# Sunscreen-tech/spf

Measured on NVIDIA B200. Metric: circuit_bootstraps_per_sec, higher is better.
Workload: dtype f64

## Files before the change

### spf_b200/csrc/kernels.cuh

```cuda
#pragma once
#include <cuda_runtime.h>

#include "team_ops.cuh"

namespace spf {

__device__ __forceinline__ void tmem_ld16(uint32_t (&r)[16], uint32_t taddr);
__device__ __forceinline__ void tmem_st16(uint32_t taddr, const uint32_t (&r)[16]);
__device__ __forceinline__ void tmem_wait_ld();
__device__ __forceinline__ void tmem_wait_st();

struct DevCx {
  static constexpr bool kTmemTwiddles = false;
  int u;
  int bar;
  uint32_t rp_taddr;
  __device__ __forceinline__ void sync() const {
    asm volatile("bar.sync %0, 64;" ::"r"(bar) : "memory");
  }
  __device__ __forceinline__ void rp_store(const uint64_t (&rp)[32]) const {
#pragma unroll
    for (int c = 0; c < 4; c++) {
      uint32_t r[16];
#pragma unroll
      for (int i = 0; i < 8; i++) { r[2 * i] = (uint32_t)rp[8 * c + i]; r[2 * i + 1] = (uint32_t)(rp[8 * c + i] >> 32); }
      tmem_st16(rp_taddr + 16 * c, r);
    }
    tmem_wait_st();
  }
  __device__ __forceinline__ void rp_load(uint64_t (&rp)[32]) const {
    uint32_t r[4][16];
#pragma unroll
    for (int c = 0; c < 4; c++) tmem_ld16(r[c], rp_taddr + 16 * c);
    tmem_wait_ld();
#pragma unroll
    for (int c = 0; c < 4; c++)
#pragma unroll
      for (int i = 0; i < 8; i++) rp[8 * c + i] = ((uint64_t)r[c][2 * i + 1] << 32) | r[c][2 * i];
  }
};

struct DevTables {
  const C2* T1;
  const C2* T2;
};

__device__ __forceinline__ void load_tables(C2* sT1, C2* sT2, const DevTables& t) {
  for (int i = threadIdx.x; i < kT1Elems; i += blockDim.x) sT1[i] = t.T1[i];
  for (int i = threadIdx.x; i < kT2Elems; i += blockDim.x) sT2[i] = t.T2[i];
  __syncthreads();
}

constexpr int kTableBytes = (kT1Elems + kT2Elems) * 16;

__device__ __forceinline__ void pdl_launch_dependents() { asm volatile("griddepcontrol.launch_dependents;" ::: "memory"); }
__device__ __forceinline__ void pdl_wait() { asm volatile("griddepcontrol.wait;" ::: "memory"); }
__device__ __forceinline__ void prefetch_l2(const void* p) { asm volatile("prefetch.global.L2 [%0];" ::"l"(p)); }

#ifndef SPF_PBS_PAIRS
#define SPF_PBS_PAIRS 3
#endif
#ifndef SPF_PBS_TRANSIENT
#define SPF_PBS_TRANSIENT 1
#endif
#ifndef SPF_PBS_TWOBUF
#define SPF_PBS_TWOBUF 0
#endif
constexpr int kPbsPairs = SPF_PBS_PAIRS;
constexpr int kPbsPairBytes = (SPF_PBS_TRANSIENT ? 0 : 2 * kN * 8) + (SPF_PBS_TWOBUF ? 4 : 2) * kXBuf * 16;
constexpr int kPbsTmemOwn0 = 64;
constexpr int kPbsTmemF0 = kPbsTmemOwn0 + 64 * kPbsPairs;
constexpr int kPbsTmemFPairs = (512 - kPbsTmemF0) / 64 < kPbsPairs ? (512 - kPbsTmemF0) / 64 : kPbsPairs;
constexpr int kPbsFParkBytes = (kPbsPairs - kPbsTmemFPairs) * 2 * kTeam * 16 * 16;
#ifndef SPF_PBS_RING
#define SPF_PBS_RING (!SPF_PBS_TWOBUF)
#endif
static_assert(!SPF_PBS_RING || SPF_PBS_TRANSIENT, "the BSK ring lives in the shared memory the transient accumulator frees");
#ifndef SPF_PBS_RING_STAGES
#define SPF_PBS_RING_STAGES 3
#endif
constexpr int kRingStages = SPF_PBS_RING_STAGES;
constexpr int kRingChunkElems = 2 * kM;
constexpr int kRingChunkBytes = kRingChunkElems * 16;
constexpr bool kPbsTablesInRing = SPF_PBS_RING && kRingStages == 4;
#ifndef SPF_PBS_PAIR_SHIFT
#define SPF_PBS_PAIR_SHIFT 0
#endif
constexpr int kPbsPairOff = (kPbsTablesInRing ? 0 : kTableBytes) + SPF_PBS_PAIR_SHIFT;
constexpr int kPbsRingOff = kPbsPairOff + kPbsPairs * kPbsPairBytes + kPbsFParkBytes;
constexpr int kPbsTablesOff = kPbsTablesInRing ? kPbsRingOff + 3 * kRingChunkBytes : 0;
constexpr int kPbsRingBytes = SPF_PBS_RING ? kRingStages * kRingChunkBytes + 64 : 0;
constexpr int kPbsSmem = kPbsRingOff + kPbsRingBytes;
static_assert(kPbsSmem <= 232448, "pbs_kernel shared memory");

#ifndef SPF_PBS_TMEM_T1
#define SPF_PBS_TMEM_T1 1
#endif
#ifndef SPF_PBS_TMEM_T2
#define SPF_PBS_TMEM_T2 1
#endif
#ifndef SPF_PBS_TMEM_F
#define SPF_PBS_TMEM_F 1
#endif
#ifndef SPF_PBS_TMEM_OWN
#define SPF_PBS_TMEM_OWN 1
#endif

__device__ __forceinline__ void tmem_ld16(uint32_t (&r)[16], uint32_t taddr) {
  asm volatile(
      "tcgen05.ld.sync.aligned.32x32b.x16.b32 {%0, %1, %2, %3, %4, %5, %6, %7, %8, %9, %10, %11, %12, %13, %14, %15}, [%16];"
      : "=r"(r[0]), "=r"(r[1]), "=r"(r[2]), "=r"(r[3]), "=r"(r[4]), "=r"(r[5]), "=r"(r[6]), "=r"(r[7]), "=r"(r[8]),
        "=r"(r[9]), "=r"(r[10]), "=r"(r[11]), "=r"(r[12]), "=r"(r[13]), "=r"(r[14]), "=r"(r[15])
      : "r"(taddr));
}
__device__ __forceinline__ void tmem_st4(uint32_t taddr, uint32_t a, uint32_t b, uint32_t c, uint32_t d) {
  asm volatile("tcgen05.st.sync.aligned.32x32b.x4.b32 [%0], {%1, %2, %3, %4};" ::"r"(taddr), "r"(a), "r"(b), "r"(c), "r"(d)
               : "memory");
}
__device__ __forceinline__ void tmem_st2(uint32_t taddr, uint32_t a, uint32_t b) {
  asm volatile("tcgen05.st.sync.aligned.32x32b.x2.b32 [%0], {%1, %2};" ::"r"(taddr), "r"(a), "r"(b) : "memory");
}
__device__ __forceinline__ void tmem_wait_ld() { asm volatile("tcgen05.wait::ld.sync.aligned;" ::: "memory"); }
__device__ __forceinline__ void tmem_wait_st() { asm volatile("tcgen05.wait::st.sync.aligned;" ::: "memory"); }

constexpr int kPbsTmemCols = 512;
__device__ __forceinline__ void tmem_ld8(uint32_t (&r)[8], uint32_t taddr) {
  asm volatile("tcgen05.ld.sync.aligned.32x32b.x8.b32 {%0, %1, %2, %3, %4, %5, %6, %7}, [%8];"
               : "=r"(r[0]), "=r"(r[1]), "=r"(r[2]), "=r"(r[3]), "=r"(r[4]), "=r"(r[5]), "=r"(r[6]), "=r"(r[7])
               : "r"(taddr));
}
__device__ __forceinline__ void tmem_st8(uint32_t taddr, const uint32_t (&r)[8]) {
  asm volatile("tcgen05.st.sync.aligned.32x32b.x8.b32 [%0], {%1, %2, %3, %4, %5, %6, %7, %8};" ::"r"(taddr), "r"(r[0]), "r"(r[1]),
               "r"(r[2]), "r"(r[3]), "r"(r[4]), "r"(r[5]), "r"(r[6]), "r"(r[7])
               : "memory");
}
__device__ __forceinline__ void tmem_st16(uint32_t taddr, const uint32_t (&r)[16]) {
  asm volatile(
      "tcgen05.st.sync.aligned.32x32b.x16.b32 [%0], {%1, %2, %3, %4, %5, %6, %7, %8, %9, %10, %11, %12, %13, %14, %15, %16};"
      ::"r"(taddr), "r"(r[0]), "r"(r[1]), "r"(r[2]), "r"(r[3]), "r"(r[4]), "r"(r[5]), "r"(r[6]), "r"(r[7]), "r"(r[8]),
        "r"(r[9]), "r"(r[10]), "r"(r[11]), "r"(r[12]), "r"(r[13]), "r"(r[14]), "r"(r[15])
      : "memory");
}

__device__ __forceinline__ uint32_t smem_u32(const void* p) { return (uint32_t)__cvta_generic_to_shared(p); }
__device__ __forceinline__ void mbar_wait_trap(uint32_t bar, uint32_t parity) {
  unsigned long long t_start = 0;
  for (int spin = 0;; spin++) {
    uint32_t ok;
#if SPF_MBAR_HINT
    asm volatile("{\n\t.reg .pred p;\n\tmbarrier.try_wait.parity.shared::cta.b64 p, [%1], %2, %3;\n\tselp.u32 %0, 1, 0, p;\n\t}"
                 : "=r"(ok) : "r"(bar), "r"(parity), "r"((uint32_t)SPF_MBAR_HINT) : "memory");
#else
    asm volatile("{\n\t.reg .pred p;\n\tmbarrier.try_wait.parity.shared::cta.b64 p, [%1], %2;\n\tselp.u32 %0, 1, 0, p;\n\t}"
                 : "=r"(ok) : "r"(bar), "r"(parity) : "memory");
#endif
    if (ok) return;
    if ((spin & 1023) == 1023) {
      unsigned long long now;
      asm volatile("mov.u64 %0, %%globaltimer;" : "=l"(now));
      if (t_start == 0) t_start = now;
      else if (now - t_start > 2000000000ull) __trap();
    }
  }
}
static_assert(!SPF_PBS_TRANSIENT || SPF_PBS_TMEM_OWN, "the transient accumulator image needs the tensor-memory own copy");
static_assert(!kPbsTablesInRing || SPF_PBS_TMEM_T1, "four ring stages overlay the twiddle tables: the twiddles must live in tensor memory");

#ifndef SPF_PBS_CHUNKED
#define SPF_PBS_CHUNKED 1
#endif
#ifndef SPF_PBS_READER_T2
#define SPF_PBS_READER_T2 1
#endif
#ifndef SPF_PBS_INT_CONV
#define SPF_PBS_INT_CONV 0
#endif
#ifndef SPF_PBS_FST2
#define SPF_PBS_FST2 1
#endif
#ifndef SPF_PBS_EARLY_REL
#define SPF_PBS_EARLY_REL 0
#endif
#ifndef SPF_PBS_RING_FENCE
#define SPF_PBS_RING_FENCE 1
#endif
#ifndef SPF_MBAR_HINT
#define SPF_MBAR_HINT 0
#endif
#ifndef SPF_PBS_FRND_CONV
#define SPF_PBS_FRND_CONV 0
#endif
#ifndef SPF_PBS_TW_PIPE
#define SPF_PBS_TW_PIPE 0
#endif
#ifndef SPF_PBS_FUSED_ST
#define SPF_PBS_FUSED_ST 0
#endif
#ifndef SPF_PBS_TMEM_X1
#define SPF_PBS_TMEM_X1 0
#endif
__device__ __forceinline__ void tmem_ld256x4(uint32_t* r, uint32_t taddr) {
  asm volatile(
      "tcgen05.ld.sync.aligned.16x256b.x4.b32 {%0, %1, %2, %3, %4, %5, %6, %7, %8, %9, %10, %11, %12, %13, %14, %15}, [%16];"
      : "=r"(r[0]), "=r"(r[1]), "=r"(r[2]), "=r"(r[3]), "=r"(r[4]), "=r"(r[5]), "=r"(r[6]), "=r"(r[7]), "=r"(r[8]),
        "=r"(r[9]), "=r"(r[10]), "=r"(r[11]), "=r"(r[12]), "=r"(r[13]), "=r"(r[14]), "=r"(r[15])
      : "r"(taddr));
}
__device__ __forceinline__ void tmem_st256x4(uint32_t taddr, const uint32_t* r) {
  asm volatile(
      "tcgen05.st.sync.aligned.16x256b.x4.b32 [%0], {%1, %2, %3, %4, %5, %6, %7, %8, %9, %10, %11, %12, %13, %14, %15, %16};"
      ::"r"(taddr), "r"(r[0]), "r"(r[1]), "r"(r[2]), "r"(r[3]), "r"(r[4]), "r"(r[5]), "r"(r[6]), "r"(r[7]), "r"(r[8]),
        "r"(r[9]), "r"(r[10]), "r"(r[11]), "r"(r[12]), "r"(r[13]), "r"(r[14]), "r"(r[15])
      : "memory");
}
__device__ __forceinline__ void tmem_ld16p(uint32_t* r, uint32_t taddr) {
  asm volatile(
      "tcgen05.ld.sync.aligned.32x32b.x16.b32 {%0, %1, %2, %3, %4, %5, %6, %7, %8, %9, %10, %11, %12, %13, %14, %15}, [%16];"
      : "=r"(r[0]), "=r"(r[1]), "=r"(r[2]), "=r"(r[3]), "=r"(r[4]), "=r"(r[5]), "=r"(r[6]), "=r"(r[7]), "=r"(r[8]),
        "=r"(r[9]), "=r"(r[10]), "=r"(r[11]), "=r"(r[12]), "=r"(r[13]), "=r"(r[14]), "=r"(r[15])
      : "r"(taddr));
}
__device__ __forceinline__ void tmem_st16p(uint32_t taddr, const uint32_t* r) {
  asm volatile(
      "tcgen05.st.sync.aligned.32x32b.x16.b32 [%0], {%1, %2, %3, %4, %5, %6, %7, %8, %9, %10, %11, %12, %13, %14, %15, %16};"
      ::"r"(taddr), "r"(r[0]), "r"(r[1]), "r"(r[2]), "r"(r[3]), "r"(r[4]), "r"(r[5]), "r"(r[6]), "r"(r[7]), "r"(r[8]),
        "r"(r[9]), "r"(r[10]), "r"(r[11]), "r"(r[12]), "r"(r[13]), "r"(r[14]), "r"(r[15])
      : "memory");
}
__device__ __forceinline__ constexpr int x1_unit1(int k, int c) { return (k >> 2) + 4 * (c + 2 * (k & 3)); }
__device__ __forceinline__ constexpr int x1_unit2(int e, int klo, int c) { return klo + 4 * (c + 2 * e); }
__device__ __forceinline__ constexpr int x1_reg256(int b, int eh, int ch, int cg, int w) { return 16 * (2 * b + ch) + w + 2 * eh + 4 * cg; }
__device__ __forceinline__ constexpr int x1_reg_r1(int e, int klo, int c, int w) {
  return x1_reg256(e >> 1, e & 1, klo >> 1, c + 2 * (klo & 1), w);
}
__device__ __forceinline__ constexpr int x1_reg_r2(int e, int ep, int c, int w) {
  return x1_reg256(ep >> 1, ep & 1, e >> 1, c + 2 * (e & 1), w);
}
__device__ __forceinline__ void x1_ld256(uint32_t (&r)[64], uint32_t ta) {
  tmem_ld256x4(r, ta); tmem_ld256x4(r + 16, ta + 32); tmem_ld256x4(r + 32, ta + (16u << 16)); tmem_ld256x4(r + 48, ta + 32 + (16u << 16));
}
__device__ __forceinline__ void x1_st256(uint32_t ta, const uint32_t (&r)[64]) {
  tmem_st256x4(ta, r); tmem_st256x4(ta + 32, r + 16); tmem_st256x4(ta + (16u << 16), r + 32); tmem_st256x4(ta + 32 + (16u << 16), r + 48);
}
__device__ __forceinline__ void x1_ld32(uint32_t (&r)[64], uint32_t ta) {
  tmem_ld16p(r, ta); tmem_ld16p(r + 16, ta + 16); tmem_ld16p(r + 32, ta + 32); tmem_ld16p(r + 48, ta + 48);
}
__device__ __forceinline__ void x1_st32(uint32_t ta, const uint32_t (&r)[64]) {
  tmem_st16p(ta, r); tmem_st16p(ta + 16, r + 16); tmem_st16p(ta + 32, r + 32); tmem_st16p(ta + 48, r + 48);
}
struct DevPairCx {
  static constexpr bool kTransient = SPF_PBS_TRANSIENT != 0;
  static constexpr bool kChunked = SPF_PBS_CHUNKED != 0;
  static constexpr bool kFusedStores = SPF_PBS_FUSED_ST != 0;
  static __device__ __forceinline__ void sts_c2(C2* p, C2 v) {
    asm volatile("st.shared.v2.f64 [%0], {%1, %2};" ::"r"((uint32_t)__cvta_generic_to_shared(p)), "d"(v.x), "d"(v.y) : "memory");
  }
  __device__ __forceinline__ void sts(C2* p, C2 v) const { sts_c2(p, v); }
  template <bool CONJ>
  __device__ __forceinline__ void t1_mul_store(C2 (&v)[16], const C2* T1, C2* buf) const {
#pragma unroll
    for (int g = 0; g < 4; g++) {
      uint32_t r[16];
      tmem_ld16(r, t1_taddr + 16 * g);
      tmem_wait_ld();
#pragma unroll
      for (int i = 0; i < 4; i++) {
        const C2 w{__hiloint2double((int)r[4 * i + 1], (int)r[4 * i]), __hiloint2double((int)r[4 * i + 3], (int)r[4 * i + 2])};
        const int k = 4 * g + i;
        v[k] = CONJ ? cmul_conj(v[k], w) : cmul(v[k], w);
        sts_c2(buf + k * kXPad + u, v[k]);
      }
    }
  }
  template <bool CONJ>
  __device__ __forceinline__ void t2_mul_store(C2 (&v)[16], const C2* T2, C2* buf) const {
    const int k1 = u & 15, q = u >> 4;
#pragma unroll
    for (int k2 = 0; k2 < 16; k2++) {
      if (k2) v[k2] = CONJ ? cmul_conj(v[k2], T2[q * kT2Pad + k2]) : cmul(v[k2], T2[q * kT2Pad + k2]);
      sts_c2(buf + k1 * kXPad + q + 4 * k2, v[k2]);
    }
  }
  static constexpr bool kTmemX1 = SPF_PBS_TMEM_X1 != 0;
  __device__ __forceinline__ int time_index() const { return kTmemX1 ? x1_time_index(u) : u; }
  __device__ __forceinline__ void x1_fwd(C2 (&v)[16]) const {
    uint32_t r[64], s[64];
#pragma unroll
    for (int k = 0; k < 16; k++) {
      r[2 * x1_unit1(k, 0)] = (uint32_t)__double2loint(v[k].x); r[2 * x1_unit1(k, 0) + 1] = (uint32_t)__double2hiint(v[k].x);
      r[2 * x1_unit1(k, 1)] = (uint32_t)__double2loint(v[k].y); r[2 * x1_unit1(k, 1) + 1] = (uint32_t)__double2hiint(v[k].y);
    }
    x1_st32(f_taddr, r);
    tmem_wait_st();
    x1_ld256(s, f_taddr);
    tmem_wait_ld();
#pragma unroll
    for (int e = 0; e < 4; e++)
#pragma unroll
      for (int klo = 0; klo < 4; klo++)
#pragma unroll
        for (int c = 0; c < 2; c++)
#pragma unroll
          for (int w = 0; w < 2; w++) r[2 * x1_unit2(e, klo, c) + w] = s[x1_reg_r1(e, klo, c, w)];
    x1_st32(f_taddr, r);
    tmem_wait_st();
    x1_ld256(s, f_taddr);
    tmem_wait_ld();
#pragma unroll
    for (int e = 0; e < 4; e++)
#pragma unroll
      for (int ep = 0; ep < 4; ep++) {
        v[4 * e + ep].x = __hiloint2double((int)s[x1_reg_r2(e, ep, 0, 1)], (int)s[x1_reg_r2(e, ep, 0, 0)]);
        v[4 * e + ep].y = __hiloint2double((int)s[x1_reg_r2(e, ep, 1, 1)], (int)s[x1_reg_r2(e, ep, 1, 0)]);
      }
  }
// ... 1721 lines not shown
```

### spf_b200/csrc/team_ops.cuh

```cuda
#pragma once
#include <type_traits>

#include "fft16.cuh"

namespace spf {

constexpr double kInvM = 1.0 / 1024.0;

SPF_HD C2 ldg_c2(const C2* p) {
#if defined(__CUDA_ARCH__)
  const double2 t = __ldg(reinterpret_cast<const double2*>(p));
  return C2{t.x, t.y};
#else
  return *p;
#endif
}
SPF_HD C2 ldg_c2_pinned(const C2* p) {
#if defined(__CUDA_ARCH__)
  C2 r;
  asm volatile("ld.global.v2.f64 {%0, %1}, [%2];" : "=d"(r.x), "=d"(r.y) : "l"(p) : "memory");
  return r;
#else
  return *p;
#endif
// ... 83 lines not shown
#pragma unroll
  for (int m = 0; m < 16; m++) {
    v[m].x = i64_to_f64((int64_t)coef(cx.u + 64 * m));
    v[m].y = i64_to_f64((int64_t)coef(cx.u + 64 * m + kM));
  }
  team_fft_fwd(cx, v, xbuf, T1, T2);
#pragma unroll
  for (int s = 0; s < 16; s++) { v[s].x *= kInvM; v[s].y *= kInvM; }
}

template <class Cx, class F>
SPF_HD void state_init(Cx& cx, uint64_t* st, int radix_log, int count, F coef) {
#pragma unroll 4
  for (int i = 0; i < 32; i++) st[i * 64 + cx.u] = radix_round(coef(cx.u + 64 * i), radix_log, count);
}

template <class Cx>
SPF_HD void gadget_mad(Cx& cx, C2 (&acc)[2][16], uint64_t* st, C2* xbuf, const C2* T1, const C2* T2,
                       const C2* glev, int radix_log, int count) {
  for (int t = 0; t < count; t++) {
    C2 v[16];
#pragma unroll
    for (int m = 0; m < 16; m++) {
      uint64_t s0 = st[m * 64 + cx.u], s1 = st[(m + 16) * 64 + cx.u];
      v[m].x = i32_to_f64(next_digit(s0, radix_log));
      v[m].y = i32_to_f64(next_digit(s1, radix_log));
      st[m * 64 + cx.u] = s0;
      st[(m + 16) * 64 + cx.u] = s1;
    }
    team_fft_fwd(cx, v, xbuf, T1, T2);
    mad_glwe(acc, v, glev + (size_t)(count - 1 - t) * 2 * kM, cx.u);
  }
}

template <class Cx, class F>
SPF_HD void gadget_mad_stateless(Cx& cx, C2 (&acc)[2][16], F coef, C2* xbuf, const C2* T1, const C2* T2, const C2* glev,
                                 int radix_log, int count) {
  const uint64_t off = radix_offset(radix_log, count);
  const uint64_t dmask = (1ull << radix_log) - 1;
  const int32_t half = 1 << (radix_log - 1);
  {
    uint64_t rp[32];
#pragma unroll
    for (int i2 = 0; i2 < 32; i2++) rp[i2] = radix_round(coef(cx.u + 64 * i2), radix_log, count) + off;
    cx.rp_store(rp);
  }
  for (int t = 0; t < count; t++) {
    C2 v[16];
    {
      uint64_t rp[32];
      cx.rp_load(rp);
#pragma unroll
      for (int m = 0; m < 16; m++) {
        v[m].x = i32_to_f64((int32_t)((rp[m] >> (t * radix_log)) & dmask) - half);
        v[m].y = i32_to_f64((int32_t)((rp[m + 16] >> (t * radix_log)) & dmask) - half);
      }
    }
    team_fft_fwd(cx, v, xbuf, T1, T2);
    mad_glwe(acc, v, glev + (size_t)(count - 1 - t) * 2 * kM, cx.u);
  }
}

template <class Cx>
SPF_HD void cmux_team(Cx& cx, uint64_t* out, const uint64_t* d0, const uint64_t* d1, const C2* ggsw,
                      uint64_t* st, C2* xbuf, const C2* T1, const C2* T2, int radix_log, int count) {
  C2 acc[2][16];
  zero_acc(acc);
  for (int r = 0; r < 2; r++) {
    const uint64_t* a1 = d1 + r * kN;
    const uint64_t* a0 = d0 ? d0 + r * kN : nullptr;
    state_init(cx, st, radix_log, count,
               [&](int j) { return a0 ? ldg_u64(a1 + j) - ldg_u64(a0 + j) : ldg_u64(a1 + j); });
    gadget_mad(cx, acc, st, xbuf, T1, T2, ggsw + (size_t)r * count * 2 * kM, radix_log, count);
  }
#pragma unroll
  for (int p = 0; p < 2; p++) {
    team_fft_inv(cx, acc[p], xbuf, T1, T2);
#pragma unroll
    for (int m = 0; m < 16; m++) {
      const int j = cx.u + 64 * m;
      uint64_t re = f64_to_torus(acc[p][m].x), im = f64_to_torus(acc[p][m].y);
      if (d0) { re += ldg_u64(d0 + p * kN + j); im += ldg_u64(d0 + p * kN + j + kM); }
      out[p * kN + j] = re;
      out[p * kN + j + kM] = im;
    }
  }
}

struct PbsArgs {
  const uint64_t* lwe_in;
  const uint64_t* lut;
  uint64_t* glwe_out;
  const C2* bsk;
  int lwe_n;
  int log_chi, log_v;
  int cbs_radix_log, cbs_count;
};

SPF_HD uint32_t modulus_switch(uint64_t x, int log_chi, int log_v, int log_modulus) {
  const uint64_t mask = (1ull << log_modulus) - 1;
  x <<= log_chi;
  const int shift = 64 - (log_modulus - log_v);
  const uint64_t rnd = (x >> (shift - 1)) & 1;
  x >>= shift;
  return (uint32_t)(((x + rnd) & mask) << log_v);
}

SPF_HD uint64_t cbs_lut_coeff(int idx, int cbs_radix_log, int cbs_count, int v) {
  const int f = idx & (v - 1);
  if (f >= cbs_count) return 0;
  const int pb = cbs_radix_log * (f + 1) + 1;
  return pb < 64 ? 0 - (1ull << (64 - pb)) : 0;
}

template <bool INIT>
SPF_HD void mad_poly(C2 (&acc)[16], const C2 (&v)[16], const C2* g, int u) {
#pragma unroll
  for (int h = 0; h < 4; h++) {
    C2 b[4];
#pragma unroll
    for (int i = 0; i < 4; i++) b[i] = ldg_c2(g + bin_of(u, 4 * h + i));
#pragma unroll
    for (int i = 0; i < 4; i++) {
      if (INIT) acc[4 * h + i] = cmul(v[4 * h + i], b[i]);
      else cmad(acc[4 * h + i], v[4 * h + i], b[i]);
    }
  }
}
SPF_HD void mad_poly_shared(C2 (&acc)[16], const C2* dbuf, const C2* g, int u) {
#pragma unroll
  for (int h = 0; h < 4; h++) {
    C2 b[4], d[4];
#pragma unroll
    for (int i = 0; i < 4; i++) {
      b[i] = ldg_c2(g + bin_of(u, 4 * h + i));
      d[i] = dbuf[(4 * h + i) * 64 + u];
    }
#pragma unroll
    for (int i = 0; i < 4; i++) cmad(acc[4 * h + i], d[i], b[i]);
  }
}

SPF_HD double digit16_to_f64(uint32_t d) {
  const uint64_t bits = 0x4330000000000000ull | (uint64_t)((d & 0xFFFFu) ^ 0x8000u);
  double x;
#if defined(__CUDA_ARCH__)
  x = __longlong_as_double((long long)bits);
#else
  __builtin_memcpy(&x, &bits, 8);
#endif
  return x - 4503599627403264.0;
}

#ifndef SPF_GATHER_SEL
#define SPF_GATHER_SEL 0
#endif
#ifndef SPF_DIGIT_I2F
#define SPF_DIGIT_I2F 1
#endif
SPF_HD double digit_lo16_to_f64(uint32_t d) {
#if defined(__CUDA_ARCH__) && SPF_DIGIT_I2F
  double r;
  asm("{\n\t.reg .b16 lo, hi;\n\tmov.b32 {lo, hi}, %1;\n\tcvt.rn.f64.s16 %0, lo;\n\t}" : "=d"(r) : "r"(d));
  return r;
#else
  return bits_f64(0x4230000000000000ull | (uint64_t)(uint32_t)(d * 65536u + 0x80000000u)) - 68719509504.0;
#endif
}
SPF_HD double digit_hi16_to_f64(uint32_t d) {
#if defined(__CUDA_ARCH__) && SPF_DIGIT_I2F
  double r;
  asm("{\n\t.reg .b16 lo, hi;\n\tmov.b32 {lo, hi}, %1;\n\tcvt.rn.f64.s16 %0, hi;\n\t}" : "=d"(r) : "r"(d));
  return r;
#else
  return bits_f64(0x4230000000000000ull | (uint64_t)(uint32_t)((d & 0xFFFF0000u) ^ 0x80000000u)) - 68719509504.0;
#endif
}


SPF_HD constexpr int split_bin(int u, int h, int s) { return u + 64 * (2 * h + (s >> 2) + 4 * (s & 3)); }

template <bool INIT, class Cx>
SPF_HD void mad_split(Cx& cx, C2 (&f)[2][8], const C2* xbb, const C2* g , int u, int h) {
  const int k1 = u & 15, q = u >> 4;
#pragma unroll
  for (int jj = 0; jj < 2; jj++) {
    C2 d[4], g0[4], g1[4];
#pragma unroll
    for (int qp = 0; qp < 4; qp++) d[qp] = SPF_ABLATE(4) ? C2{1.0 + qp, 2.0 + jj} : xbb[k1 * kXPad + qp + 4 * q + 16 * (2 * h + jj)];
#pragma unroll
    for (int k3 = 0; k3 < 4; k3++) {
      g0[k3] = cx.bsk_load(g + split_bin(u, h, 4 * jj + k3));
      g1[k3] = cx.bsk_load(g + kM + split_bin(u, h, 4 * jj + k3));
    }
    bfly4<false>(d[0], d[1], d[2], d[3]);
#pragma unroll
    for (int k3 = 0; k3 < 4; k3++) {
      const int s = 4 * jj + k3;
      if (INIT) { f[0][s] = cmul(d[k3], g0[k3]); f[1][s] = cmul(d[k3], g1[k3]); }
      else { cmad(f[0][s], d[k3], g0[k3]); cmad(f[1][s], d[k3], g1[k3]); }
    }
  }
}

SPF_HD void rt2_fwd_consts(const C2* T2, int q, int h, double (&o)[12]) {
  for (int jj = 0; jj < 2; jj++) {
    const int k2 = q + 4 * (2 * h + jj);
    double c[4];
    for (int qp = 1; qp < 4; qp++) {
      const C2 w = T2[qp * kT2Pad + k2];
      c[qp] = w.x == 0.0 ? 8.470329472543003e-22  : w.x;
      o[6 * jj + qp - 1] = w.y / c[qp];
    }
    o[6 * jj + 3] = c[1];
    o[6 * jj + 4] = c[2];
    o[6 * jj + 5] = c[3] / c[1];
  }
}
SPF_HD void rt2_inv_consts(const C2* T2, int q, int h, C2 (&o)[6]) {
  for (int jj = 0; jj < 2; jj++)
    for (int qp = 1; qp < 4; qp++) o[3 * jj + qp - 1] = T2[qp * kT2Pad + q + 4 * (2 * h + jj)];
}
SPF_HD void rt2_group_consts(const C2* T2, int q, int grp, double (&tw)[6], C2 (&wi)[3]) {
  const int k2 = q + 4 * grp;
  double c[4];
  for (int qp = 1; qp < 4; qp++) {
    const C2 w = T2[qp * kT2Pad + k2];
    wi[qp - 1] = w;
    c[qp] = w.x == 0.0 ? 8.470329472543003e-22  : w.x;
    tw[qp - 1] = w.y / c[qp];
  }
  tw[3] = c[1];
  tw[4] = c[2];
  tw[5] = c[3] / c[1];
}
template <bool INIT, class Cx>
SPF_HD void mad_split_rt(Cx& cx, C2 (&f)[2][8], const C2* xbb, const C2* g, int u, int h, const double (&tw)[12]) {
  const int k1 = u & 15, q = u >> 4;
#pragma unroll
  for (int jj = 0; jj < 2; jj++) {
    C2 d[4], g0[4], g1[4];
#pragma unroll
    for (int qp = 0; qp < 4; qp++) d[qp] = SPF_ABLATE(4) ? C2{1.0 + qp, 2.0 + jj} : xbb[k1 * kXPad + qp + 4 * q + 16 * (2 * h + jj)];
#pragma unroll
    for (int k3 = 0; k3 < 4; k3++) {
      g0[k3] = cx.bsk_load(g + split_bin(u, h, 4 * jj + k3));
      g1[k3] = cx.bsk_load(g + kM + split_bin(u, h, 4 * jj + k3));
    }
#pragma unroll
    for (int qp = 1; qp < 4; qp++) {
      const double t = tw[6 * jj + qp - 1];
      if (SPF_ABLATE(2)) d[qp] = abl_mix(d[qp], C2{t, t});
      else d[qp] = C2{spf_fma(-t, d[qp].y, d[qp].x), spf_fma(t, d[qp].x, d[qp].y)};
    }
    bfly4_r<false>(d[0], d[1], d[2], d[3], tw[6 * jj + 3], tw[6 * jj + 4], tw[6 * jj + 5]);
#pragma unroll
    for (int k3 = 0; k3 < 4; k3++) {
      const int s = 4 * jj + k3;
      if (INIT) { f[0][s] = cmul(d[k3], g0[k3]); f[1][s] = cmul(d[k3], g1[k3]); }
      else { cmad(f[0][s], d[k3], g0[k3]); cmad(f[1][s], d[k3], g1[k3]); }
    }
  }
}

template <class Cx>
SPF_HD void pbs_pair_team(Cx& cx, const PbsArgs& A, uint64_t* acc, C2* xb, const C2* T1, const C2* T2, int& G) {
  const int u = cx.u, h = cx.h;
  const int k1 = u & 15, q = u >> 4;
  const int n = A.lwe_n;
  const bool cbs = A.lut == nullptr;
  const int log2n = 12;
  C2* xown = xb + h * kXBuf;
  constexpr bool kX1 = Cx::kTmemX1;
  const int ua = cx.time_index();
  constexpr bool kTr = Cx::kTransient;
  uint64_t* pa = kTr ? reinterpret_cast<uint64_t*>(xown) : acc + h * kN;
  {
    uint64_t b = ldg_u64(A.lwe_in + n);
    if (cbs) b += 1ull << 62;
    const int bt = (int)modulus_switch(b, A.log_chi, A.log_v, log2n);
    const int rot = (2 * kN - bt) & (2 * kN - 1);
    const int v = 1 << A.log_v;
    for (int i = 0; i < 32; i++) {
      const int j = ua + 64 * i;
      int idx = j - rot;
      bool neg = false;
      if (idx < 0) { idx += kN; neg = true; }
      if (idx < 0) { idx += kN; neg = false; }
      uint64_t c;
      if (cbs) c = h ? cbs_lut_coeff(idx, A.cbs_radix_log, A.cbs_count, v) : 0;
      else c = ldg_u64(A.lut + h * kN + idx);
      pa[u + 64 * i] = neg ? 0 - c : c;
    }
  }
  cx.sync();
  uint64_t a_next = n > 0 ? ldg_u64(A.lwe_in) : 0;
  constexpr bool kCh = Cx::kChunked;
  uint64_t own[kCh ? 8 : 32];
  {
    uint64_t o0[32];
#pragma unroll
    for (int i2 = 0; i2 < 32; i2++) o0[i2] = pa[u + 64 * i2];
    cx.own_store(o0);
    if constexpr (!kCh) {
#pragma unroll
      for (int i2 = 0; i2 < 32; i2++) own[i2] = o0[i2];
    }
  }
#pragma unroll 1
  for (int i = 0; i < n; i++) {
    const int at = (int)modulus_switch(a_next, A.log_chi, A.log_v, log2n);
    if (i + 1 < n) a_next = ldg_u64(A.lwe_in + i + 1);
    if (at == 0) {
      cx.bsk_skip(G);
      G += 4;
      continue;
    }
    const C2* ggsw = A.bsk + (size_t)i * 8 * kM;
    C2 f[2][8];
    {
      C2 v[16];
      uint32_t pk[16];
      {
        const int base = (ua - at) & (2 * kN - 1);
        const char* col = reinterpret_cast<const char*>(pa) + 8 * (kX1 ? x1_position(base & 63) : (base & 63));
        const uint32_t bh9 = (uint32_t)(base >> 6) << 9;
#if SPF_GATHER_SEL
        const int rb = (base >> 6) & 31;
        const int wrap = 32 - rb;
        const char* pU = col + 512 * rb;
        const char* pW = pU - 32 * 512;
        const uint32_t mU = 0u - (uint32_t)(base >> 11), mW = ~mU;
#endif
#pragma unroll
        for (int i2 = 0; i2 < 32; i2++) {
          if constexpr (kCh) {
            if ((i2 & 7) == 0) cx.own_ld8(own, i2 >> 3);
          }
#if SPF_GATHER_SEL
          const bool wr = i2 >= wrap;
          const uint64_t xr = *reinterpret_cast<const uint64_t*>((wr ? pW : pU) + 512 * i2);
          const uint32_t m = wr ? mW : mU;
          const uint64_t mm = ((uint64_t)m << 32) | m;
          const uint64_t diff = ((xr ^ mm) - mm) - own[kCh ? (i2 & 7) : i2];
#else
          const uint32_t t9 = bh9 + 512u * i2;
          const uint64_t x = SPF_ABLATE(32) ? (uint64_t)t9 * 0x9E3779B97F4A7C15ull : *reinterpret_cast<const uint64_t*>(col + (t9 & 0x3E00u));
          const uint64_t diff = ((t9 & 0x4000u) ? 0 - x : x) - own[kCh ? (i2 & 7) : i2];
#endif
          const uint32_t w = (uint32_t)(diff >> 32) + ((uint32_t)diff >> 31);
          const uint32_t w1 = w + 0x8000u;
          if (i2 < 16) { v[i2].x = digit_lo16_to_f64(w); pk[i2] = w1 >> 16; }
          else { v[i2 - 16].y = digit_lo16_to_f64(w); pk[i2 - 16] |= w1 & 0xFFFF0000u; }
        }
      }
      if constexpr (Cx::kTwoBuf) {
        static_assert(!Cx::kBskRing && !Cx::kTmemX1 && !Cx::kFusedStores && Cx::kReaderT2, "two-buffer form: LDG key, reader-side pass-2 twiddles");
        C2* xown2 = xb + (2 + h) * kXBuf;
        fwd_pass1_core(v);
        cx.template t1_mul<false>(v, T1);
        if (kTr) cx.sync();
        fwd_x1_write(v, xown, u);
#pragma unroll
        for (int m = 0; m < 16; m++) { v[m].x = digit_lo16_to_f64(pk[m]); v[m].y = digit_hi16_to_f64(pk[m]); }
        fwd_pass1_core(v);
        cx.template t1_mul<false>(v, T1);
        fwd_x1_write(v, xown2, u);
        cx.sync();
        fwd_x1_read(v, xown, u);
        dft16<false>(v);
        fwd_x2_write(v, xown, u);
        fwd_x1_read(v, xown2, u);
        dft16<false>(v);
        fwd_x2_write(v, xown2, u);
        cx.pair_sync();
        double tw[12];
        cx.rt2_fwd(tw, T2);
        mad_split_rt<true>(cx, f, xb, ggsw + (size_t)((0 * 2 + 1) * 2) * kM, u, h, tw);
        mad_split_rt<false>(cx, f, xb + kXBuf, ggsw + (size_t)((1 * 2 + 1) * 2) * kM, u, h, tw);
        mad_split_rt<false>(cx, f, xb + 2 * kXBuf, ggsw + (size_t)((0 * 2 + 0) * 2) * kM, u, h, tw);
        mad_split_rt<false>(cx, f, xb + 3 * kXBuf, ggsw + (size_t)((1 * 2 + 0) * 2) * kM, u, h, tw);
      } else {
#pragma unroll
      for (int t = 0; t < 2; t++) {
        const int level = 1 - t;
        if (t == 1) {
#pragma unroll
          for (int m = 0; m < 16; m++) { v[m].x = digit_lo16_to_f64(pk[m]); v[m].y = digit_hi16_to_f64(pk[m]); }
        }
        fwd_pass1_core(v);
        if constexpr (Cx::kFusedStores) {
          if (t == 1) { cx.pair_sync(); cx.bsk_release(G); cx.bsk_release(G + 1); }
          else if (kTr) cx.sync();
          cx.template t1_mul_store<false>(v, T1, xown);
          cx.sync();
          fwd_x1_read(v, xown, u);
          dft16<false>(v);
          if constexpr (Cx::kReaderT2) fwd_x2_write(v, xown, u);
          else cx.template t2_mul_store<false>(v, T2, xown);
        } else {
          cx.template t1_mul<false>(v, T1);
          if constexpr (kX1) {
            if (t == 0) {
              cx.x1_fwd(v);
              dft16<false>(v);
              if constexpr (!Cx::kReaderT2) cx.template t2_mul<false>(v, T2);
              if (kTr) cx.sync();
            } else {
              cx.pair_sync(); cx.bsk_release(G); cx.bsk_release(G + 1);
              fwd_x1_write(v, xown, u);
              cx.sync();
              fwd_x1_read_perm(v, xown, u);
              dft16<false>(v);
              if constexpr (!Cx::kReaderT2) cx.template t2_mul<false>(v, T2);
              cx.sync();
            }
            fwd_x2_write(v, xown, u);
          } else {
          if (t == 1) { cx.pair_sync(); cx.bsk_release(G); cx.bsk_release(G + 1); }
          else if (kTr) cx.sync();
          fwd_x1_write(v, xown, u);
          cx.sync();
          fwd_x1_read(v, xown, u);
          dft16<false>(v);
          if constexpr (!Cx::kReaderT2) cx.template t2_mul<false>(v, T2);
          fwd_x2_write(v, xown, u);
          }
        }
        if (t == 1) cx.f_load(f);
        cx.pair_sync();
        const C2* g0 = cx.bsk_acquire(G + 2 * t, ggsw + (size_t)((0 * 2 + level) * 2) * kM);
        if constexpr (Cx::kReaderT2) {
          double tw[12];
          cx.rt2_fwd(tw, T2);
          if (t == 0) mad_split_rt<true>(cx, f, xb, g0, u, h, tw);
          else mad_split_rt<false>(cx, f, xb, g0, u, h, tw);
          cx.bsk_release_early(G + 2 * t);
          const C2* g1 = cx.bsk_acquire(G + 2 * t + 1, ggsw + (size_t)((1 * 2 + level) * 2) * kM);
          mad_split_rt<false>(cx, f, xb + kXBuf, g1, u, h, tw);
          cx.bsk_release_early(G + 2 * t + 1);
        } else {
        if (t == 0) mad_split<true>(cx, f, xb, g0, u, h);
        else mad_split<false>(cx, f, xb, g0, u, h);
        const C2* g1 = cx.bsk_acquire(G + 2 * t + 1, ggsw + (size_t)((1 * 2 + level) * 2) * kM);
        mad_split<false>(cx, f, xb + kXBuf, g1, u, h);
        }
        if (t == 0) cx.f_store(f);
      }
      }
    }
#pragma unroll
    for (int p = 0; p < 2; p++) {
      bfly4<true>(f[p][0], f[p][1], f[p][2], f[p][3]);
      bfly4<true>(f[p][4], f[p][5], f[p][6], f[p][7]);
    }
    if constexpr (Cx::kReaderT2) {
      C2 wi[6];
      cx.rt2_inv(wi, T2);
#pragma unroll
      for (int p = 0; p < 2; p++)
#pragma unroll
        for (int jj = 0; jj < 2; jj++)
#pragma unroll
          for (int qp = 1; qp < 4; qp++) f[p][4 * jj + qp] = cmul_conj(f[p][4 * jj + qp], wi[3 * jj + qp - 1]);
    }
#pragma unroll
    for (int p = 0; p < 2; p++) {
#pragma unroll
      for (int jj = 0; jj < 2; jj++) {
#pragma unroll
        for (int qp = 0; qp < 4; qp++)
          if (!SPF_ABLATE(4)) xb[p * kXBuf + k1 * kXPad + qp + 4 * q + 16 * (2 * h + jj)] = f[p][4 * jj + qp];
      }
    }
    cx.pair_sync();
    cx.bsk_release(G + 2);
    cx.bsk_release(G + 3);
    G += 4;
    {
      C2 w[16];
      inv_x2_read(w, xown, u);
      if constexpr (!Cx::kReaderT2) cx.template t2_mul<true>(w, T2);
      if constexpr (Cx::kFusedStores) {
        dft16_emit<true>(w, [&](int mp, C2 val) { cx.sts(xown + k1 * kXPad + q + 4 * mp, val); });
      } else if constexpr (kX1) {
        dft16<true>(w);
        cx.x1_inv(w);
      } else {
        dft16<true>(w);
        inv_x1_write(w, xown, u);
      }
      if constexpr (!kX1) {
        cx.sync();
        inv_x1_read(w, xown, u);
      }
      if (kTr) cx.sync();
      cx.template t1_mul<true>(w, T1);
      double ws[16];
      inv_pass1_core_s(w, ws);
      if constexpr (!kCh) cx.own_load(own, pa);
#pragma unroll
      for (int m4 = 0; m4 < 16; m4 += 4) {
        uint32_t mag_max = 0;
        uint64_t r[8];
        if constexpr (Cx::kFrndConv) {
          uint32_t small_min = 0x7FFFFFFFu;
#pragma unroll
          for (int i = 0; i < 4; i++) {
            r[2 * i] = f64_to_torus_frnd(w[m4 + i].x, ws[m4 + i], small_min, mag_max);
            r[2 * i + 1] = f64_to_torus_frnd(w[m4 + i].y, ws[m4 + i], small_min, mag_max);
          }
          if (__builtin_expect(small_min < kTorusSmallMag || mag_max >= kTorusHalfMag, 0)) {
#pragma unroll
            for (int i = 0; i < 4; i++) {
              r[2 * i] = f64_to_torus(ws[m4 + i] * w[m4 + i].x);
              r[2 * i + 1] = f64_to_torus(ws[m4 + i] * w[m4 + i].y);
            }
          }
        } else if constexpr (Cx::kIntConv) {
#pragma unroll
          for (int i = 0; i < 4; i++) {
            r[2 * i] = f64_to_torus_int(w[m4 + i].x, ws[m4 + i], mag_max);
            r[2 * i + 1] = f64_to_torus_int(w[m4 + i].y, ws[m4 + i], mag_max);
          }
          if (__builtin_expect(mag_max != 0, 0)) {
#pragma unroll
            for (int i = 0; i < 4; i++) {
              r[2 * i] = f64_to_torus(ws[m4 + i] * w[m4 + i].x);
              r[2 * i + 1] = f64_to_torus(ws[m4 + i] * w[m4 + i].y);
            }
          }
        } else {
#pragma unroll
        for (int i = 0; i < 4; i++) {
          r[2 * i] = f64_to_torus_s_fast(w[m4 + i].x, ws[m4 + i], mag_max);
          r[2 * i + 1] = f64_to_torus_s_fast(w[m4 + i].y, ws[m4 + i], mag_max);
        }
        if (__builtin_expect(mag_max == kTorusCornerMag, 0)) {
#pragma unroll
          for (int i = 0; i < 4; i++) {
            r[2 * i] = f64_to_torus_s(w[m4 + i].x, ws[m4 + i]);
            r[2 * i + 1] = f64_to_torus_s(w[m4 + i].y, ws[m4 + i]);
          }
        }
        }
        if constexpr (kCh) {
          cx.own_ld4x2(own, m4);
#pragma unroll
          for (int i = 0; i < 4; i++) {
            const int j = u + 64 * (m4 + i);
            own[i] += r[2 * i];
            own[4 + i] += r[2 * i + 1];
            pa[j] = own[i];
            pa[j + kM] = own[4 + i];
          }
          cx.own_st4x2(own, m4);
        } else {
#pragma unroll
          for (int i = 0; i < 4; i++) {
            const int m = m4 + i, j = u + 64 * m;
            own[m] += r[2 * i];
            own[m + 16] += r[2 * i + 1];
            pa[j] = own[m];
            pa[j + kM] = own[m + 16];
          }
        }
      }
      if constexpr (kCh) cx.own_st_wait();
      else cx.own_store(own);
    }
    cx.sync();
  }
  for (int i = 0; i < 32; i++) A.glwe_out[h * kN + ua + 64 * i] = pa[u + 64 * i];
  if (kTr) cx.sync();
}

template <class Cx>
SPF_HD void pbs_quad_team(Cx& cx, const PbsArgs& A, uint64_t* acc, C2* xb, const C2* T1, const C2* T2, int& executed) {
  const int u = cx.u, h = cx.h, t = cx.t, g = 2 * h + t;
  const int k1 = u & 15, q = u >> 4;
  const int n = A.lwe_n;
  const bool cbs = A.lut == nullptr;
  const int log2n = 12;
  uint64_t* pa = acc + h * kN;
  C2* xown = xb + g * kXBuf;
#if defined(SPF_QUAD_TRACE) && defined(__CUDA_ARCH__)
  long long qt[10] = {0, 0, 0, 0, 0, 0, 0, 0, 0, 0}, qc = 0, qn = 0;
#define SPF_QT(k) do { const long long now_ = clock64(); qt[k] += now_ - qc; qc = now_; } while (0)
#else
#define SPF_QT(k) do { } while (0)
#endif
  {
    uint64_t b = ldg_u64(A.lwe_in + n);
    if (cbs) b += 1ull << 62;
    const int bt = (int)modulus_switch(b, A.log_chi, A.log_v, log2n);
    const int rot = (2 * kN - bt) & (2 * kN - 1);
    const int v = 1 << A.log_v;
    for (int i = 16 * t; i < 16 * t + 16; i++) {
      const int j = u + 64 * i;
      int idx = j - rot;
      bool neg = false;
      if (idx < 0) { idx += kN; neg = true; }
      if (idx < 0) { idx += kN; neg = false; }
      uint64_t c;
      if (cbs) c = h ? cbs_lut_coeff(idx, A.cbs_radix_log, A.cbs_count, v) : 0;
      else c = ldg_u64(A.lut + h * kN + idx);
      pa[j] = neg ? 0 - c : c;
    }
  }
  cx.quad_sync();
  uint64_t a_next = n > 0 ? ldg_u64(A.lwe_in) : 0;
  uint64_t own[32];
#pragma unroll
  for (int i2 = 0; i2 < 32; i2++) own[i2] = pa[u + 64 * i2];
  auto next_executed = [&](int from) {
    int j = from;
    while (j < n && modulus_switch(ldg_u64(A.lwe_in + j), A.log_chi, A.log_v, log2n) == 0) j++;
    return j;
  };
  {
    const int j0 = next_executed(0);
    if (j0 < n) cx.row_prefetch(A.bsk + (size_t)j0 * 8 * kM);
  }
#pragma unroll 1
  for (int i = 0; i < n; i++) {
    const int at = (int)modulus_switch(a_next, A.log_chi, A.log_v, log2n);
    if (i + 1 < n) a_next = ldg_u64(A.lwe_in + i + 1);
    if (at == 0) continue;
    const C2* ggsw = A.bsk + (size_t)i * 8 * kM;
#if defined(SPF_QUAD_TRACE) && defined(__CUDA_ARCH__)
    qc = clock64(); qn++;
#endif
    {
      C2 v[16];
      const int base = (u - at) & (2 * kN - 1);
      const char* col = reinterpret_cast<const char*>(pa) + 8 * (base & 63);
      const uint32_t bh9 = (uint32_t)(base >> 6) << 9;
      if constexpr (Cx::kSplitGather) {
        uint32_t pk[8];
        auto gather_half = [&](auto tt) {
          constexpr int T = decltype(tt)::value;
#pragma unroll
          for (int k = 0; k < 16; k++) {
            const int i2 = 16 * T + k;
            const uint32_t t9 = bh9 + 512u * i2;
            const uint64_t x = *reinterpret_cast<const uint64_t*>(col + (t9 & 0x3E00u));
            const uint64_t diff = ((t9 & 0x4000u) ? 0 - x : x) - own[i2];
            const uint32_t w = (uint32_t)(diff >> 32) + ((uint32_t)diff >> 31);
            const uint32_t w1 = w + 0x8000u;
            const uint32_t other = T ? (w & 0xFFFFu) : (w1 >> 16);
            if (T) v[k].y = digit_hi16_to_f64(w1); else v[k].x = digit_lo16_to_f64(w);
            if (k & 1) pk[k >> 1] |= other << 16; else pk[k >> 1] = other;
          }
        };
        if (t) gather_half(std::integral_constant<int, 1>{}); else gather_half(std::integral_constant<int, 0>{});
        cx.digit_xchg(pk);
#pragma unroll
        for (int k = 0; k < 16; k++) {
          const double d = digit_lo16_to_f64(pk[k >> 1] >> (16 * (k & 1)));
          if (t) v[k].x = d; else v[k].y = d;
        }
      } else {
#pragma unroll
      for (int i2 = 0; i2 < 32; i2++) {
        const uint32_t t9 = bh9 + 512u * i2;
        const uint64_t x = *reinterpret_cast<const uint64_t*>(col + (t9 & 0x3E00u));
        const uint64_t diff = ((t9 & 0x4000u) ? 0 - x : x) - own[i2];
        const uint32_t w = (uint32_t)(diff >> 32) + ((uint32_t)diff >> 31);
        const double d = t ? digit_hi16_to_f64(w + 0x8000u) : digit_lo16_to_f64(w);
        if (i2 < 16) v[i2].x = d; else v[i2 - 16].y = d;
      }
      }
      SPF_QT(0);
      fwd_pass1_core(v);
      cx.template t1_mul<false>(v, T1);
      fwd_x1_write(v, xown, u);
      cx.sync();
      SPF_QT(1);
      fwd_x1_read(v, xown, u);
      dft16<false>(v);
      if constexpr (!Cx::kReaderT2) cx.template t2_mul<false>(v, T2);
      fwd_x2_write(v, xown, u);
      SPF_QT(2);
    }
    cx.quad_sync();
    SPF_QT(3);
    const C2* staged = cx.row_wait(executed, ggsw);
    executed++;
    SPF_QT(4);
    C2 f[2][4];
    double rtw[6];
    C2 rwi[3];
    if constexpr (Cx::kReaderT2) cx.rt2(rtw, rwi, T2);
#pragma unroll
    for (int b = 0; b < 4; b++) {
      const C2* grow = staged + (size_t)(((b >> 1) * 2 + (1 - (b & 1))) * 2) * kM;
      C2 d[4], g0[4], g1[4];
#pragma unroll
      for (int qp = 0; qp < 4; qp++) d[qp] = xb[b * kXBuf + k1 * kXPad + qp + 4 * q + 16 * g];
#pragma unroll
      for (int k3 = 0; k3 < 4; k3++) {
        g0[k3] = cx.row_load(grow + u + 64 * (g + 4 * k3));
        g1[k3] = cx.row_load(grow + kM + u + 64 * (g + 4 * k3));
      }
      if constexpr (Cx::kReaderT2) {
#pragma unroll
        for (int qp = 1; qp < 4; qp++) d[qp] = C2{spf_fma(-rtw[qp - 1], d[qp].y, d[qp].x), spf_fma(rtw[qp - 1], d[qp].x, d[qp].y)};
        bfly4_r<false>(d[0], d[1], d[2], d[3], rtw[3], rtw[4], rtw[5]);
      } else {
        bfly4<false>(d[0], d[1], d[2], d[3]);
// ... 355 lines not shown
```

Measured before the change: 57770.

## Streamline mbarrier wait, branchless gather via shared addressing, defer exact torus fallback

Three separate micro-optimisations. The mbarrier wait now does one fast-path try_wait and only reads the global timer in the slow loop. The rotated accumulator gather always uses the select-based form with raw 32-bit shared addresses and an xor/add negation, and packs the high digit halves with a single byte_perm. The rare exact torus conversion fallback in the chunked path is moved after the stores as a corrective delta update, taking it off the common path at the cost of an extra store-wait and re-store when the fallback triggers.

```diff
diff --git a/spf_b200/csrc/kernels.cuh b/spf_b200/csrc/kernels.cuh
--- a/spf_b200/csrc/kernels.cuh
+++ b/spf_b200/csrc/kernels.cuh
@@ -143,24 +143,25 @@
 }
 
 __device__ __forceinline__ uint32_t smem_u32(const void* p) { return (uint32_t)__cvta_generic_to_shared(p); }
+__device__ __forceinline__ bool mbar_try_wait(uint32_t bar, uint32_t parity) {
+  uint32_t ok;
+#if SPF_MBAR_HINT
+  asm volatile("{\n\t.reg .pred p;\n\tmbarrier.try_wait.parity.shared::cta.b64 p, [%1], %2, %3;\n\tselp.u32 %0, 1, 0, p;\n\t}"
+               : "=r"(ok) : "r"(bar), "r"(parity), "r"((uint32_t)SPF_MBAR_HINT) : "memory");
+#else
+  asm volatile("{\n\t.reg .pred p;\n\tmbarrier.try_wait.parity.shared::cta.b64 p, [%1], %2;\n\tselp.u32 %0, 1, 0, p;\n\t}"
+               : "=r"(ok) : "r"(bar), "r"(parity) : "memory");
+#endif
+  return ok != 0;
+}
 __device__ __forceinline__ void mbar_wait_trap(uint32_t bar, uint32_t parity) {
-  unsigned long long t_start = 0;
-  for (int spin = 0;; spin++) {
-    uint32_t ok;
-#if SPF_MBAR_HINT
-    asm volatile("{\n\t.reg .pred p;\n\tmbarrier.try_wait.parity.shared::cta.b64 p, [%1], %2, %3;\n\tselp.u32 %0, 1, 0, p;\n\t}"
-                 : "=r"(ok) : "r"(bar), "r"(parity), "r"((uint32_t)SPF_MBAR_HINT) : "memory");
-#else
-    asm volatile("{\n\t.reg .pred p;\n\tmbarrier.try_wait.parity.shared::cta.b64 p, [%1], %2;\n\tselp.u32 %0, 1, 0, p;\n\t}"
-                 : "=r"(ok) : "r"(bar), "r"(parity) : "memory");
-#endif
-    if (ok) return;
-    if ((spin & 1023) == 1023) {
-      unsigned long long now;
-      asm volatile("mov.u64 %0, %%globaltimer;" : "=l"(now));
-      if (t_start == 0) t_start = now;
-      else if (now - t_start > 2000000000ull) __trap();
-    }
+  if (__builtin_expect(mbar_try_wait(bar, parity), 1)) return;
+  unsigned long long t_start;
+  asm volatile("mov.u64 %0, %%globaltimer;" : "=l"(t_start));
+  while (!mbar_try_wait(bar, parity)) {
+    unsigned long long now;
+    asm volatile("mov.u64 %0, %%globaltimer;" : "=l"(now));
+    if (now - t_start > 2000000000ull) __trap();
   }
 }
 static_assert(!SPF_PBS_TRANSIENT || SPF_PBS_TMEM_OWN, "the transient accumulator image needs the tensor-memory own copy");
diff --git a/spf_b200/csrc/team_ops.cuh b/spf_b200/csrc/team_ops.cuh
--- a/spf_b200/csrc/team_ops.cuh
+++ b/spf_b200/csrc/team_ops.cuh
@@ -259,9 +259,6 @@
   return x - 4503599627403264.0;
 }
 
-#ifndef SPF_GATHER_SEL
-#define SPF_GATHER_SEL 0
-#endif
 #ifndef SPF_DIGIT_I2F
 #define SPF_DIGIT_I2F 1
 #endif
@@ -281,6 +278,14 @@
   return r;
 #else
   return bits_f64(0x4230000000000000ull | (uint64_t)(uint32_t)((d & 0xFFFF0000u) ^ 0x80000000u)) - 68719509504.0;
+#endif
+}
+
+SPF_HD uint32_t hi_halves(uint32_t a, uint32_t b) {
+#if defined(__CUDA_ARCH__)
+  return __byte_perm(a, b, 0x7632);
+#else
+  return (a >> 16) | (b & 0xFFFF0000u);
 #endif
 }
 
@@ -431,34 +436,36 @@
       {
         const int base = (ua - at) & (2 * kN - 1);
         const char* col = reinterpret_cast<const char*>(pa) + 8 * (kX1 ? x1_position(base & 63) : (base & 63));
-        const uint32_t bh9 = (uint32_t)(base >> 6) << 9;
-#if SPF_GATHER_SEL
         const int rb = (base >> 6) & 31;
         const int wrap = 32 - rb;
         const char* pU = col + 512 * rb;
+#if defined(__CUDA_ARCH__)
+        const uint32_t sU = (uint32_t)__cvta_generic_to_shared(pU);
+        uint32_t sW = sU - 32 * 512;
+        asm("" : "+r"(sW));
+#else
         const char* pW = pU - 32 * 512;
+#endif
         const uint32_t mU = 0u - (uint32_t)(base >> 11), mW = ~mU;
-#endif
 #pragma unroll
         for (int i2 = 0; i2 < 32; i2++) {
           if constexpr (kCh) {
             if ((i2 & 7) == 0) cx.own_ld8(own, i2 >> 3);
           }
-#if SPF_GATHER_SEL
           const bool wr = i2 >= wrap;
-          const uint64_t xr = *reinterpret_cast<const uint64_t*>((wr ? pW : pU) + 512 * i2);
+          uint64_t x;
+#if defined(__CUDA_ARCH__)
+          asm volatile("ld.shared.u64 %0, [%1];" : "=l"(x) : "r"((wr ? sW : sU) + 512u * i2));
+#else
+          x = *reinterpret_cast<const uint64_t*>((wr ? pW : pU) + 512 * i2);
+#endif
+          if (SPF_ABLATE(32)) x = (uint64_t)(i2 + rb) * 0x9E3779B97F4A7C15ull;
           const uint32_t m = wr ? mW : mU;
-          const uint64_t mm = ((uint64_t)m << 32) | m;
-          const uint64_t diff = ((xr ^ mm) - mm) - own[kCh ? (i2 & 7) : i2];
-#else
-          const uint32_t t9 = bh9 + 512u * i2;
-          const uint64_t x = SPF_ABLATE(32) ? (uint64_t)t9 * 0x9E3779B97F4A7C15ull : *reinterpret_cast<const uint64_t*>(col + (t9 & 0x3E00u));
-          const uint64_t diff = ((t9 & 0x4000u) ? 0 - x : x) - own[kCh ? (i2 & 7) : i2];
-#endif
+          const uint64_t diff = (x ^ (((uint64_t)m << 32) | m)) + (m & 1u) - own[kCh ? (i2 & 7) : i2];
           const uint32_t w = (uint32_t)(diff >> 32) + ((uint32_t)diff >> 31);
           const uint32_t w1 = w + 0x8000u;
-          if (i2 < 16) { v[i2].x = digit_lo16_to_f64(w); pk[i2] = w1 >> 16; }
-          else { v[i2 - 16].y = digit_lo16_to_f64(w); pk[i2 - 16] |= w1 & 0xFFFF0000u; }
+          if (i2 < 16) { v[i2].x = digit_lo16_to_f64(w); pk[i2] = w1; }
+          else { v[i2 - 16].y = digit_lo16_to_f64(w); pk[i2 - 16] = hi_halves(pk[i2 - 16], w1); }
         }
       }
       if constexpr (Cx::kTwoBuf) {
@@ -610,6 +617,7 @@
       for (int m4 = 0; m4 < 16; m4 += 4) {
         uint32_t mag_max = 0;
         uint64_t r[8];
+        bool redo;
         if constexpr (Cx::kFrndConv) {
           uint32_t small_min = 0x7FFFFFFFu;
 #pragma unroll
@@ -617,40 +625,27 @@
             r[2 * i] = f64_to_torus_frnd(w[m4 + i].x, ws[m4 + i], small_min, mag_max);
             r[2 * i + 1] = f64_to_torus_frnd(w[m4 + i].y, ws[m4 + i], small_min, mag_max);
           }
-          if (__builtin_expect(small_min < kTorusSmallMag || mag_max >= kTorusHalfMag, 0)) {
-#pragma unroll
-            for (int i = 0; i < 4; i++) {
-              r[2 * i] = f64_to_torus(ws[m4 + i] * w[m4 + i].x);
-              r[2 * i + 1] = f64_to_torus(ws[m4 + i] * w[m4 + i].y);
-            }
-          }
+          redo = small_min < kTorusSmallMag || mag_max >= kTorusHalfMag;
         } else if constexpr (Cx::kIntConv) {
 #pragma unroll
           for (int i = 0; i < 4; i++) {
             r[2 * i] = f64_to_torus_int(w[m4 + i].x, ws[m4 + i], mag_max);
             r[2 * i + 1] = f64_to_torus_int(w[m4 + i].y, ws[m4 + i], mag_max);
           }
-          if (__builtin_expect(mag_max != 0, 0)) {
-#pragma unroll
-            for (int i = 0; i < 4; i++) {
-              r[2 * i] = f64_to_torus(ws[m4 + i] * w[m4 + i].x);
-              r[2 * i + 1] = f64_to_torus(ws[m4 + i] * w[m4 + i].y);
-            }
+          redo = mag_max != 0;
+        } else {
+#pragma unroll
+          for (int i = 0; i < 4; i++) {
+            r[2 * i] = f64_to_torus_s_fast(w[m4 + i].x, ws[m4 + i], mag_max);
+            r[2 * i + 1] = f64_to_torus_s_fast(w[m4 + i].y, ws[m4 + i], mag_max);
           }
-        } else {
-#pragma unroll
-        for (int i = 0; i < 4; i++) {
-          r[2 * i] = f64_to_torus_s_fast(w[m4 + i].x, ws[m4 + i], mag_max);
-          r[2 * i + 1] = f64_to_torus_s_fast(w[m4 + i].y, ws[m4 + i], mag_max);
+          redo = mag_max == kTorusCornerMag;
         }
-        if (__builtin_expect(mag_max == kTorusCornerMag, 0)) {
-#pragma unroll
-          for (int i = 0; i < 4; i++) {
-            r[2 * i] = f64_to_torus_s(w[m4 + i].x, ws[m4 + i]);
-            r[2 * i + 1] = f64_to_torus_s(w[m4 + i].y, ws[m4 + i]);
-          }
-        }
-        }
+        auto exact = [&](int k) -> uint64_t {
+          const double x = (k & 1) ? w[m4 + (k >> 1)].y : w[m4 + (k >> 1)].x;
+          if constexpr (Cx::kFrndConv || Cx::kIntConv) return f64_to_torus(ws[m4 + (k >> 1)] * x);
+          else return f64_to_torus_s(x, ws[m4 + (k >> 1)]);
+        };
         if constexpr (kCh) {
           cx.own_ld4x2(own, m4);
 #pragma unroll
@@ -662,7 +657,23 @@
             pa[j + kM] = own[4 + i];
           }
           cx.own_st4x2(own, m4);
+          if (__builtin_expect(redo, 0)) {
+            cx.own_st_wait();
+#pragma unroll
+            for (int i = 0; i < 4; i++) {
+              const int j = u + 64 * (m4 + i);
+              own[i] += exact(2 * i) - r[2 * i];
+              own[4 + i] += exact(2 * i + 1) - r[2 * i + 1];
+              pa[j] = own[i];
+              pa[j + kM] = own[4 + i];
+            }
+            cx.own_st4x2(own, m4);
+          }
         } else {
+          if (__builtin_expect(redo, 0)) {
+#pragma unroll
+            for (int k = 0; k < 8; k++) r[k] = exact(k);
+          }
 #pragma unroll
           for (int i = 0; i < 4; i++) {
             const int m = m4 + i, j = u + 64 * m;
```

Measured after the change: 59440, median of 6. 1.03x the previous value.
